# psychopa4/PFNL

Measured on AMD Instinct MI355X. Metric: HR frames/sec at 4xSR, 7-frame 128x128->512x512, higher is better.
Workload: dtype f32

## Files before the change

### pfnl_amd/csrc/nonlocal_f16.hip

```cpp
#include <algorithm>
#include <cstdlib>
#include <type_traits>

#include "common.h"
#include "conv_bf16.h"
#include "conv_split16.h"

namespace pfnl {

typedef _Float16 bf16x8 __attribute__((ext_vector_type(8)));
typedef unsigned u32x4 __attribute__((ext_vector_type(4)));

constexpr int NF_KT = 64;
constexpr int NF_KROW = 208;
constexpr int NF_VROW = 144;
constexpr int NF_CP = 96;
constexpr int NF_THREADS = 512;
constexpr int NF_QB = NF_THREADS / 2;

constexpr float NF_XSCALE = 128.0f;
constexpr float NF_SINV = 1.0f / (128.0f * 128.0f);
constexpr float NF_PSHIFT = 14.0f;
__device__ __forceinline__ unsigned short bf16_bits(float f) {
    const _Float16 b = (_Float16)f;
    return __builtin_bit_cast(unsigned short, b);
}
__device__ __forceinline__ float bf16_float(unsigned short u) { return (float)__builtin_bit_cast(_Float16, u); }

template <bool FROMX>
__global__ __launch_bounds__(256) void nl_pack_f16_kernel(const float* __restrict__ X, uint16_t* __restrict__ Khi, uint16_t* __restrict__ Klo,
                                                          uint16_t* __restrict__ Vthi, uint16_t* __restrict__ Vtlo, int B, int N, int Npad, int C,
                                                          int CPin, const float* __restrict__ xraw, float* __restrict__ Xout, int H, int W) {
    __shared__ uint16_t vth[NF_CP][34], vtl[NF_CP][34];
    const int nblk = Npad / 32;
    const int b = blockIdx.x / nblk, n0 = (blockIdx.x - b * nblk) * 32;
    const int tid = threadIdx.x;
    [[maybe_unused]] const int C3 = C / 4, T = C / 12, W2 = W / 2;
#pragma unroll
    for (int j = 0; j < 32 * NF_CP / 256; ++j) {
        const int i = tid + 256 * j;
        const int kk = i / NF_CP, c = i - kk * NF_CP;
        const int n = n0 + kk;
        float raw = 0.f;
        if constexpr (FROMX) {
            if (n < N && c < C) {
                const int sub = c / C3, k = c - sub * C3;
                const int t = k / 3, cc = k - 3 * t;
                const int y = 2 * (n / W2) + (sub >> 1), xx = 2 * (n % W2) + (sub & 1);
                raw = xraw[((((size_t)b * T + t) * H + y) * W + xx) * 3 + cc];
            }
            if (n < N && c < CPin) Xout[((size_t)b * N + n) * CPin + c] = raw;
        } else {
            raw = (n < N && c < C) ? X[((size_t)b * N + n) * CPin + c] : 0.f;
        }
        const float v = raw * NF_XSCALE;
        const unsigned short hi = bf16_bits(v);
        const unsigned short lo = bf16_bits(v - bf16_float(hi));
        Khi[((size_t)b * Npad + n) * NF_CP + c] = (n >= N && c == C) ? (unsigned short)0xfbff : (c == C + 1 ? (unsigned short)0x3c00 : hi);
        Klo[((size_t)b * Npad + n) * NF_CP + c] = lo;
        const int e = (kk & 3) | (((kk >> 3) & 1) << 2), kh = (kk >> 2) & 1, t = kk >> 4;
        const int pos = 16 * t + 8 * kh + e;
        vth[c][pos] = c == C ? (unsigned short)0x3c00 : hi;
        vtl[c][pos] = c == C ? (unsigned short)0 : lo;
    }
    __syncthreads();
#pragma unroll
    for (int j = 0; j < 16 * NF_CP / 256; ++j) {
        const int i = tid + 256 * j;
        const int c = i >> 4, pp = (i & 15) * 2;
        const size_t vp = ((size_t)b * NF_CP + c) * Npad + n0 + pp;
        *reinterpret_cast<unsigned*>(Vthi + vp) = (unsigned)vth[c][pp] | ((unsigned)vth[c][pp + 1] << 16);
        *reinterpret_cast<unsigned*>(Vtlo + vp) = (unsigned)vtl[c][pp] | ((unsigned)vtl[c][pp + 1] << 16);
    }
}



template <bool SPLIT>
struct NfSW {
    static constexpr int KLO_OFF = NF_KT * NF_KROW;
    static constexpr int VHI_OFF = SPLIT ? 2 * NF_KT * NF_KROW : NF_KT * NF_KROW;
    static constexpr int VLO_OFF = VHI_OFF + NF_CP * NF_VROW;
    static constexpr int TILE_BYTES = SPLIT ? VLO_OFF + NF_CP * NF_VROW : VLO_OFF;
    static constexpr int NSLOT = SPLIT ? 3 : 5;
    static constexpr int PIECES = SPLIT ? 53 : 32;
    static constexpr int SLOT_BYTES = PIECES * 1024;
    static constexpr int PW = (PIECES + 7) / 8;
    static constexpr int LDS_BYTES = NSLOT * SLOT_BYTES;
    static_assert(TILE_BYTES <= SLOT_BYTES && LDS_BYTES <= 160 * 1024, "LDS budget");
    static_assert(SPLIT || PIECES % 8 == 0, "the vmcnt wait of a ring deeper than 3 counts on equal shares");
};

__device__ __forceinline__ void nf_dma16(__amdgpu_buffer_rsrc_t rs, unsigned lds_dst, int voff) {
    unsigned keep;
    asm volatile("s_mov_b32 %0, m0\n\ts_mov_b32 m0, %2\n\ts_nop 0\n\tbuffer_load_dwordx4 %1, %3, 0 offen lds\n\ts_mov_b32 m0, %0"
                 : "=&s"(keep) : "v"(voff), "s"(lds_dst), "s"(rs) : "memory");
}
#define NF_BARRIER() asm volatile("s_waitcnt lgkmcnt(0)\n\ts_barrier" ::: "memory")

template <int C, bool SPLIT>
__global__ __launch_bounds__(NF_THREADS, 2) void nl_attn_f16_sw_kernel(const float* __restrict__ X, const uint16_t* __restrict__ K16,
                                                                 unsigned rel_klo, unsigned rel_vhi, unsigned rel_vlo, unsigned scratch_bytes,
                                                                 float* __restrict__ Xo, const float* __restrict__ Wp,
                                                                 const float* __restrict__ bp, float* __restrict__ Zp,
                                                                 float* __restrict__ ML, int N, int Npad, int q0, int q1) {
    using G = NfSW<SPLIT>;
    constexpr int CT = 3;
    constexpr int CP = (C + 31) / 32 * 32;
    static_assert(C + 1 < NF_CP && C % 2 == 0, "needs two pad channels inside 96");
    extern __shared__ __attribute__((aligned(16))) unsigned char sm[];

    const int tid = threadIdx.x;
    const int lane = tid & 63;
    const int wave = __builtin_amdgcn_readfirstlane(tid >> 6);
    const int xl = lane & 31;
    const int kh = lane >> 5;
    const int b = blockIdx.y;
    const float* Xb = X + (size_t)b * N * CP;
    float* Xob = Xo + (size_t)b * N * CP;
    const int q = q0 + blockIdx.x * NF_QB + (tid >> 6) * 32 + xl;
    const int qc = q < q1 ? q : q1 - 1;

    constexpr float LOG2E = 1.4426950408889634f;
    bf16x8 qh[6];
    [[maybe_unused]] bf16x8 ql[6];
#pragma unroll
    for (int ks = 0; ks < 6; ++ks)
#pragma unroll
        for (int e = 0; e < 8; ++e) {
            const int c = 16 * ks + 8 * kh + e;
            const float v = c < C ? Xb[(size_t)qc * CP + c] * (LOG2E * NF_XSCALE) : (c == C ? 1024.f : 0.f);
            const _Float16 h = (_Float16)v;
            qh[ks][e] = h;
            if constexpr (SPLIT) ql[ks][e] = (_Float16)(v - (float)h);
        }
    constexpr int CS = C;
    constexpr int LCT = CS / 32, LI = CS % 32;
    constexpr int LKH = (LI % 8) >= 4 ? 1 : 0, LR = (LI / 8) * 4 + (LI % 8) % 4;

    f32x16 o[CT];
#pragma unroll
    for (int ct = 0; ct < CT; ++ct)
#pragma unroll
        for (int r = 0; r < 16; ++r) o[ct][r] = 0.f;
    float m = -INFINITY;

    int srel[G::PW];
#pragma unroll
    for (int k = 0; k < G::PW; ++k) {
        const int p = (wave + 8 * k) * 1024 + 16 * lane;
        int sr = 0x7fffffff;
        if (p < NF_KT * NF_KROW || (SPLIT && p < 2 * NF_KT * NF_KROW)) {
            const bool lo = p >= NF_KT * NF_KROW;
            const int r = p - (lo ? NF_KT * NF_KROW : 0);
            const int row = r / NF_KROW, col = r - row * NF_KROW;
            if (col < NF_CP * 2) {
                sr = (int)((lo ? rel_klo : 0u) + (unsigned)(((size_t)b * Npad + row) * (NF_CP * 2)) + col);
            }
        } else if (p < G::TILE_BYTES) {
            const bool lo = SPLIT && p >= G::VLO_OFF;
            const int r = p - (lo ? G::VLO_OFF : G::VHI_OFF);
            const int ch = r / NF_VROW, col = r - ch * NF_VROW;
            if (col < NF_KT * 2) {
                sr = (int)((lo ? rel_vlo : rel_vhi) + (unsigned)(((size_t)b * NF_CP + ch) * Npad * 2) + col);
            }
        }
        srel[k] = sr;
    }
    const unsigned lds0 = (unsigned)(uintptr_t)sm;
    auto tile_piece = [&](int k, int kt, int slot, bool live) __attribute__((always_inline)) {
        const int i = wave + 8 * k;
        if (G::PIECES % 8 == 0 || 8 * k + 7 < G::PIECES || i < G::PIECES) {
            const __amdgpu_buffer_rsrc_t rs = __builtin_amdgcn_make_buffer_rsrc(const_cast<uint16_t*>(K16), 0, live ? scratch_bytes : 0, 0x00020000);
            const int k0 = kt * NF_KT;
            const bool isk = i * 1024 < (SPLIT ? 2 : 1) * NF_KT * NF_KROW;
            const int off = (int)((unsigned)srel[k] + (unsigned)(k0 * (isk ? NF_CP * 2 : 2)));
            nf_dma16(rs, lds0 + slot * G::SLOT_BYTES + i * 1024, off);
        }
    };

    const int ntiles = (N + NF_KT - 1) / NF_KT;
    const int ksp = gridDim.z, sp = blockIdx.z;
    const int kt0 = (int)((long long)ntiles * sp / ksp), kt1 = (int)((long long)ntiles * (sp + 1) / ksp);
#pragma unroll
    for (int j = 0; j < G::NSLOT - 1; ++j)
#pragma unroll
        for (int k = 0; k < G::PW; ++k) tile_piece(k, kt0 + j, j, kt0 + j < kt1);
#pragma unroll
    for (int k = 0; k < G::PW; ++k) tile_piece(k, 0, G::NSLOT - 1, false);
    asm volatile("s_waitcnt vmcnt(0)" ::: "memory");
    __syncthreads();

    bf16x8 pt[2][2];
    [[maybe_unused]] bf16x8 pl[2][2];
#pragma unroll
    for (int i = 0; i < 2; ++i)
#pragma unroll
        for (int j = 0; j < 2; ++j)
#pragma unroll
            for (int e = 0; e < 8; ++e) {
                pt[i][j][e] = (_Float16)0.f;
                if constexpr (SPLIT) pl[i][j][e] = (_Float16)0.f;
            }
#define NP_MFMA(a_, b_, c_) __builtin_amdgcn_mfma_f32_32x32x16_f16(a_, b_, c_, 0, 0, 0)
    f32x16 st[2];
    constexpr int NQ = SPLIT ? 18 : 6, NR = SPLIT ? 24 : 12;
#define NP_PIN(v_) asm volatile("" : "+v"(v_))
    constexpr int AHEAD = 4;
    constexpr int RING = AHEAD + 2;
    bf16x8 rb[RING];
    auto half_body = [&](auto hc, const unsigned char* qbuf, const unsigned char* vbuf, int kt_fill, int s_fill) __attribute__((always_inline)) {
        constexpr int H = decltype(hc)::value;
        f32x16& stc = st[H];
        f32x16& stn = st[H ^ 1];
        const unsigned char* const kah = qbuf + ((1 - H) * 32 + xl) * NF_KROW + kh * 16;
        const unsigned char* const vah = vbuf + G::VHI_OFF + xl * NF_VROW + kh * 16 + (1 - H) * 64;
        auto read = [&](auto qc) __attribute__((always_inline)) {
            constexpr int q = decltype(qc)::value;
            if constexpr (q < NR) {
                constexpr int d = q % RING;
                if constexpr (!SPLIT) {
                    if constexpr (q < 6) rb[d] = *reinterpret_cast<const bf16x8*>(kah + q * 32);
                    else rb[d] = *reinterpret_cast<const bf16x8*>(vah + ((q - 6) % 3) * 32 * NF_VROW + ((q - 6) / 3) * 32);
                } else {
                    if constexpr (q < 12) rb[d] = *reinterpret_cast<const bf16x8*>(kah + (q & 1) * G::KLO_OFF + (q >> 1) * 32);
                    else {
                        constexpr int u = (q - 12) >> 1, lo = (q - 12) & 1;
                        rb[d] = *reinterpret_cast<const bf16x8*>(vah + lo * (G::VLO_OFF - G::VHI_OFF) + (u % 3) * 32 * NF_VROW + (u / 3) * 32);
                    }
                }
            }
        };
        auto mfma = [&](auto ic) __attribute__((always_inline)) {
            constexpr int i = decltype(ic)::value;
            constexpr int q = SPLIT ? 2 * (i / 3) + (i % 3 == 2) : i;
            const bf16x8 a = rb[q % RING];
            if constexpr (i < NQ) {
                constexpr int ks = SPLIT ? i / 3 : i;
                bf16x8 bq = qh[ks];
                if constexpr (SPLIT) {
                    if constexpr (i % 3 == 1) bq = ql[ks];
                }
                if constexpr (i == 0) {
                    f32x16 z;
#pragma unroll
                    for (int r = 0; r < 16; ++r) z[r] = 0.f;
                    stn = NP_MFMA(a, bq, z);
                } else {
                    stn = NP_MFMA(a, bq, stn);
                }
            } else {
                constexpr int j = i - NQ;
                constexpr int u = SPLIT ? j / 3 : j;
                constexpr int jj = u / 3, ct = u % 3;
                bf16x8 bp = pt[1 - H][jj];
                if constexpr (SPLIT) {
                    if constexpr (j % 3 == 1) bp = pl[1 - H][jj];
                }
                o[ct] = NP_MFMA(a, bp, o[ct]);
            }
        };
#pragma unroll
        for (int q0_ = 0; q0_ <= AHEAD; ++q0_) {
            if (q0_ == 0) read(std::integral_constant<int, 0>{});
            if (q0_ == 1) read(std::integral_constant<int, 1>{});
            if (q0_ == 2) read(std::integral_constant<int, 2>{});
            if (q0_ == 3) read(std::integral_constant<int, 3>{});
            if (q0_ == 4) read(std::integral_constant<int, 4>{});
            if (q0_ == 5) read(std::integral_constant<int, 5>{});
            if (q0_ == 6) read(std::integral_constant<int, 6>{});
        }
        __builtin_amdgcn_sched_barrier(0);
        float tmax = 0.f, tsw = 0.f, alpha = 1.f, shift = 0.f;
        [[maybe_unused]] float pv0 = 0.f, pv1 = 0.f;
        auto gap = [&](auto ic) __attribute__((always_inline)) {
            constexpr int i = decltype(ic)::value;
            mfma(ic);
            __builtin_amdgcn_sched_barrier(0);
            {
                constexpr int qn = (SPLIT ? 2 * (i / 3) + (i % 3 == 2) : i) + AHEAD + 1;
                constexpr int qp = i == 0 ? AHEAD + 1 : (SPLIT ? 2 * ((i - 1) / 3) + ((i - 1) % 3 == 2) : i - 1) + AHEAD + 1;
                if constexpr (qn > qp) read(std::integral_constant<int, qn - 1 < NR ? (qn - 1 >= qp ? qn - 1 : NR) : NR>{});
            }
            if constexpr (i == 0) {
                float ta, tb;
                asm("v_max3_f32 %0, %1, %2, %3" : "=v"(ta) : "v"(stc[0]), "v"(stc[1]), "v"(stc[2]));
                asm("v_max3_f32 %0, %1, %2, %3" : "=v"(tb) : "v"(stc[8]), "v"(stc[9]), "v"(stc[10]));
                asm("v_max3_f32 %0, %1, %2, %3" : "=v"(ta) : "v"(ta), "v"(stc[3]), "v"(stc[4]));
                asm("v_max3_f32 %0, %1, %2, %3" : "=v"(tb) : "v"(tb), "v"(stc[11]), "v"(stc[12]));
                asm("v_max3_f32 %0, %1, %2, %3" : "=v"(ta) : "v"(ta), "v"(stc[5]), "v"(stc[6]));
                asm("v_max3_f32 %0, %1, %2, %3" : "=v"(tb) : "v"(tb), "v"(stc[13]), "v"(stc[14]));
                asm("v_max3_f32 %0, %1, %2, %3" : "=v"(ta) : "v"(ta), "v"(stc[7]), "v"(stc[15]));
                asm("v_max_f32 %0, %1, %2" : "=v"(tmax) : "v"(ta), "v"(tb));
                NP_PIN(tmax);
            } else if constexpr (i == 1) {
                tsw = __shfl_xor(tmax, 32);
                NP_PIN(tsw);
            } else if constexpr (i == 3) {
                asm("v_max_f32 %0, %1, %2" : "=v"(tmax) : "v"(tmax), "v"(tsw));
                tmax *= NF_SINV;
                const float mn = fmaxf(m, tmax);
                alpha = __builtin_amdgcn_exp2f(m - mn);
                shift = NF_PSHIFT - mn;
                m = mn;
                NP_PIN(shift);
                NP_PIN(alpha);
            }
            if constexpr (!SPLIT) {
                if constexpr (i >= 4) {
                    constexpr int r = 2 * (i - 4);
                    const float a0 = __builtin_amdgcn_exp2f(__builtin_fmaf(stc[r], NF_SINV, shift));
                    const float a1 = __builtin_amdgcn_exp2f(__builtin_fmaf(stc[r + 1], NF_SINV, shift));
                    pt[H][r >> 3][r & 7] = (_Float16)a0;
                    pt[H][r >> 3][(r & 7) + 1] = (_Float16)a1;
                    NP_PIN(pt[H][r >> 3]);
                }
            } else {
                if constexpr (i >= 4 && i % 2 == 0) {
                    constexpr int r = 2 * ((i - 4) / 4);
                    if constexpr (((i - 4) / 2) % 2 == 0) {
                        pv0 = __builtin_amdgcn_exp2f(__builtin_fmaf(stc[r], NF_SINV, shift));
                        pv1 = __builtin_amdgcn_exp2f(__builtin_fmaf(stc[r + 1], NF_SINV, shift));
                        asm volatile("" : "+v"(pv0), "+v"(pv1));
                    } else {
                        const _Float16 h0 = (_Float16)pv0, h1 = (_Float16)pv1;
                        pt[H][r >> 3][r & 7] = h0;
                        pt[H][r >> 3][(r & 7) + 1] = h1;
                        pl[H][r >> 3][r & 7] = (_Float16)(pv0 - (float)h0);
                        pl[H][r >> 3][(r & 7) + 1] = (_Float16)(pv1 - (float)h1);
                        NP_PIN(pt[H][r >> 3]);
                        NP_PIN(pl[H][r >> 3]);
                    }
                }
            }
            if constexpr (H == 1) {
                constexpr int step = SPLIT ? 5 : 3;
                if constexpr (i % step == 2 && i / step < G::PW) tile_piece(i / step, kt_fill, s_fill, kt_fill < kt1);
            }
            __builtin_amdgcn_sched_barrier(0);
        };
        gap(std::integral_constant<int, 0>{});
        gap(std::integral_constant<int, 1>{});
        gap(std::integral_constant<int, 2>{});
        gap(std::integral_constant<int, 3>{});
        gap(std::integral_constant<int, 4>{});
        gap(std::integral_constant<int, 5>{});
        gap(std::integral_constant<int, 6>{});
        gap(std::integral_constant<int, 7>{});
        gap(std::integral_constant<int, 8>{});
        gap(std::integral_constant<int, 9>{});
        gap(std::integral_constant<int, 10>{});
        gap(std::integral_constant<int, 11>{});
        if constexpr (SPLIT) {
            gap(std::integral_constant<int, 12>{});
            gap(std::integral_constant<int, 13>{});
            gap(std::integral_constant<int, 14>{});
            gap(std::integral_constant<int, 15>{});
            gap(std::integral_constant<int, 16>{});
            gap(std::integral_constant<int, 17>{});
            gap(std::integral_constant<int, 18>{});
            gap(std::integral_constant<int, 19>{});
            gap(std::integral_constant<int, 20>{});
            gap(std::integral_constant<int, 21>{});
            gap(std::integral_constant<int, 22>{});
            gap(std::integral_constant<int, 23>{});
            gap(std::integral_constant<int, 24>{});
            gap(std::integral_constant<int, 25>{});
            gap(std::integral_constant<int, 26>{});
            gap(std::integral_constant<int, 27>{});
            gap(std::integral_constant<int, 28>{});
            gap(std::integral_constant<int, 29>{});
            gap(std::integral_constant<int, 30>{});
            gap(std::integral_constant<int, 31>{});
            gap(std::integral_constant<int, 32>{});
            gap(std::integral_constant<int, 33>{});
            gap(std::integral_constant<int, 34>{});
            gap(std::integral_constant<int, 35>{});
        }
        if (!__all(alpha == 1.0f)) {
#pragma unroll
            for (int ct = 0; ct < CT; ++ct)
#pragma unroll
                for (int r = 0; r < 16; ++r) o[ct][r] *= alpha;
        }
    };

    int s_cur = 0, s_prv = G::NSLOT - 1, s_nxt = 1;
    {
        const unsigned char* const kah = sm + xl * NF_KROW + kh * 16;
#pragma unroll
        for (int r = 0; r < 16; ++r) st[0][r] = 0.f;
#pragma unroll
        for (int ks = 0; ks < 6; ++ks) {
            const bf16x8 ah = *reinterpret_cast<const bf16x8*>(kah + ks * 32);
            st[0] = NP_MFMA(ah, qh[ks], st[0]);
            if constexpr (SPLIT) {
                const bf16x8 al = *reinterpret_cast<const bf16x8*>(kah + G::KLO_OFF + ks * 32);
                st[0] = NP_MFMA(ah, ql[ks], st[0]);
                st[0] = NP_MFMA(al, qh[ks], st[0]);
            }
        }
    }
    for (int kt = kt0; kt < kt1; ++kt) {
        const unsigned char* const cur = sm + s_cur * G::SLOT_BYTES;
        const unsigned char* const prv = sm + s_prv * G::SLOT_BYTES;
        const unsigned char* const nxt = sm + s_nxt * G::SLOT_BYTES;
        half_body(std::integral_constant<int, 0>{}, cur, prv, 0, 0);
        asm volatile("s_waitcnt vmcnt(%0)" ::"n"((G::NSLOT - 3) * G::PW) : "memory");
        NF_BARRIER();
        half_body(std::integral_constant<int, 1>{}, nxt, cur, kt + G::NSLOT - 1, s_prv);
        s_prv = s_cur;
        s_cur = s_nxt;
        s_nxt = s_nxt + 1 == G::NSLOT ? 0 : s_nxt + 1;
    }
    {
        const unsigned char* const vah = sm + s_prv * G::SLOT_BYTES + G::VHI_OFF + xl * NF_VROW + kh * 16 + 64;
#pragma unroll
        for (int jj = 0; jj < 2; ++jj)
#pragma unroll
            for (int ct = 0; ct < CT; ++ct) {
                const bf16x8 vh = *reinterpret_cast<const bf16x8*>(vah + ct * 32 * NF_VROW + jj * 32);
                o[ct] = NP_MFMA(vh, pt[1][jj], o[ct]);
                if constexpr (SPLIT) {
                    const bf16x8 vl = *reinterpret_cast<const bf16x8*>(vah + (G::VLO_OFF - G::VHI_OFF) + ct * 32 * NF_VROW + jj * 32);
                    o[ct] = NP_MFMA(vh, pl[1][jj], o[ct]);
                    o[ct] = NP_MFMA(vl, pt[1][jj], o[ct]);
                }
            }
    }

    float l = o[LCT][LR];
    {
        const float lo = __shfl_xor(l, 32);
        if (kh != LKH) l = lo;
    }
    const float inv = (1.0f / NF_XSCALE) / l;
#pragma unroll
    for (int ct = 0; ct < CT; ++ct)
#pragma unroll
        for (int r = 0; r < 16; ++r) o[ct][r] *= inv;

    constexpr int CTW = CP / 32;
    constexpr int NPAIR = CTW * CTW * 2;
    static_assert(NPAIR * 2048 <= G::SLOT_BYTES * G::NSLOT, "W' in operand form fits the ring");
    asm volatile("s_waitcnt vmcnt(0)" ::: "memory");
    __syncthreads();
    for (int pp = tid; pp < NPAIR * 64; pp += NF_THREADS) {
        const int ln = pp & 63, g = pp >> 6;
        const int t = g & 1, ctp = (g >> 1) % CTW, cotp = (g >> 1) / CTW;
        const float* w = Wp + (size_t)(ctp * 32 + 16 * t + 4 * (ln >> 5)) * CP + cotp * 32 + (ln & 31);
        bf16x8 h, l;
#pragma unroll
        for (int i = 0; i < 8; ++i) {
            const float v = w[((i & 3) + 8 * (i >> 2)) * CP];
            const _Float16 hh = (_Float16)v;
            h[i] = hh;
            l[i] = (_Float16)((v - (float)hh) * 2048.0f);
        }
        *reinterpret_cast<bf16x8*>(sm + g * 2048 + ln * 16) = h;
        *reinterpret_cast<bf16x8*>(sm + g * 2048 + 1024 + ln * 16) = l;
    }
    bf16x8 bh[CTW][2], bl[CTW][2];
#pragma unroll
    for (int ct = 0; ct < CTW; ++ct)
#pragma unroll
        for (int t = 0; t < 2; ++t)
#pragma unroll
            for (int i = 0; i < 8; ++i) {
                const float v = o[ct][8 * t + i];
                const _Float16 hh = (_Float16)v;
                bh[ct][t][i] = hh;
                bl[ct][t][i] = (_Float16)((v - (float)hh) * 2048.0f);
            }
    __syncthreads();
#pragma unroll
    for (int cot = 0; cot < CTW; ++cot) {
        f32x16 z, zc;
#pragma unroll
        for (int r = 0; r < 16; ++r) z[r] = zc[r] = 0.f;
#pragma unroll
        for (int ct = 0; ct < CTW; ++ct)
#pragma unroll
            for (int t = 0; t < 2; ++t) {
                const unsigned char* wa = sm + ((cot * CTW + ct) * 2 + t) * 2048 + lane * 16;
                const bf16x8 ah = *reinterpret_cast<const bf16x8*>(wa), al = *reinterpret_cast<const bf16x8*>(wa + 1024);
                z = NP_MFMA(ah, bh[ct][t], z);
                zc = NP_MFMA(ah, bl[ct][t], zc);
                zc = NP_MFMA(al, bh[ct][t], zc);
            }
#pragma unroll
        for (int r = 0; r < 16; ++r) z[r] = (z[r] + zc[r] * (1.0f / 2048.0f)) * (ksp == 1 ? 1.0f : l);
        if (q < q1) {
            if (ksp == 1) {
#pragma unroll
                for (int r = 0; r < 16; ++r) {
                    const int co = cot * 32 + drow(r, lane);
                    if (co < C) {
                        const size_t idx = (size_t)q * CP + co;
                        Xob[idx] = Xb[idx] + z[r] + bp[co];
                    }
                }
            } else {
                float* zp = Zp + (((size_t)b * ksp + sp) * N + q) * CP;
#pragma unroll
                for (int r = 0; r < 16; ++r) zp[cot * 32 + drow(r, lane)] = z[r];
            }
        }
    }
    if (ksp > 1 && q < q1 && kh == 0) {
        float* ml = ML + (((size_t)b * ksp + sp) * N + q) * 2;
        ml[0] = m;
        ml[1] = l;
    }
}

size_t nl_f16_scratch_halfs(int B, int N) {
    const size_t npad = (size_t)(N + 31) / 32 * 32 + 64;
    return 4 * (size_t)B * NF_CP * npad;
}

static size_t nl_f16_chunk_limit() {
    static const size_t lim = [] {
        const char* e = std::getenv("PFNL_NL_CHUNK_BYTES");
        const long long v = e ? std::atoll(e) : 0;
        return v > 0 ? (size_t)v : (size_t)0x7fff0000ull;
    }();
    return lim;
}

static hipError_t nl_attn_f16_run(const float* X, float* Xo, const float* Wp, const float* bp, float* partial, uint16_t* scratch16,
                                  int B, int N, int C, hipStream_t s, int q0, int q1, bool split, int ks_cap, bool prepacked = false);

bool nl_f16_fits_one_launch(int B, int N) { return 2 * nl_f16_scratch_halfs(1, N) * (size_t)B <= nl_f16_chunk_limit(); }

hipError_t launch_nl_pack_fused(const float* x, float* X, uint16_t* scratch16, int B, int T, int H, int W, hipStream_t s) {
    const int C = 12 * T, N = (H / 2) * (W / 2);
    if (!x || !X || !scratch16 || B < 1 || (C != 84 && C != 60 && C != 36) || (H & 1) || (W & 1) || !nl_f16_fits_one_launch(B, N)) return hipErrorInvalidValue;
    const int CP = nl_padded_ch(C);
    const int npad = (N + 31) / 32 * 32 + 64;
    uint16_t* Khi = scratch16;
    uint16_t* Klo = Khi + (size_t)B * npad * NF_CP;
    uint16_t* Vthi = Klo + (size_t)B * npad * NF_CP;
    uint16_t* Vtlo = Vthi + (size_t)B * NF_CP * npad;
    hipLaunchKernelGGL(nl_pack_f16_kernel<true>, dim3(B * (npad / 32)), dim3(256), 0, s, nullptr, Khi, Klo, Vthi, Vtlo, B, N, npad, C, CP, x, X, H, W);
    return hipGetLastError();
}

hipError_t launch_nl_attn_f16(const float* X, float* Xo, const float* Wp, const float* bp, float* partial, uint16_t* scratch16,
                               int B, int N, int C, hipStream_t s, int q0, int q1, bool split, bool prepacked) {
    if (B < 1 || N < 1) return hipErrorInvalidValue;
    if (prepacked) {
        if (!nl_f16_fits_one_launch(B, N)) return hipErrorInvalidValue;
        return nl_attn_f16_run(X, Xo, Wp, bp, partial, scratch16, B, N, C, s, q0, q1, split, nl_key_splits(B, N), true);
    }
    const size_t per_clip = 2 * nl_f16_scratch_halfs(1, N);
    const int ks_cap = nl_key_splits(B, N);
    int bc = (int)std::min<size_t>((size_t)B, std::max<size_t>(1, nl_f16_chunk_limit() / per_clip));
    const int CP = nl_padded_ch(C);
    for (int b0 = 0; b0 < B; b0 += bc) {
        const int nb = std::min(bc, B - b0);
        hipError_t e = nl_attn_f16_run(X + (size_t)b0 * N * CP, Xo + (size_t)b0 * N * CP, Wp, bp, partial, scratch16, nb, N, C, s, q0, q1, split, ks_cap);
        if (e != hipSuccess) return e;
    }
    return hipSuccess;
}

static hipError_t nl_attn_f16_run(const float* X, float* Xo, const float* Wp, const float* bp, float* partial, uint16_t* scratch16,
                                  int B, int N, int C, hipStream_t s, int q0, int q1, bool split, int ks_cap, bool prepacked) {
    if (C != 84 && C != 60 && C != 36) return hipErrorInvalidValue;
    if (q1 < 0) q1 = N;
    if (q0 < 0 || q0 >= q1 || q1 > N) return hipErrorInvalidValue;
    const int CP = nl_padded_ch(C);
    const int npad = (N + 31) / 32 * 32 + 64;
    uint16_t* Khi = scratch16;
    uint16_t* Klo = Khi + (size_t)B * npad * NF_CP;
    uint16_t* Vthi = Klo + (size_t)B * npad * NF_CP;
    uint16_t* Vtlo = Vthi + (size_t)B * NF_CP * npad;
    if (!prepacked) {
        hipLaunchKernelGGL(nl_pack_f16_kernel<false>, dim3(B * (npad / 32)), dim3(256), 0, s, X, Khi, Klo, Vthi, Vtlo, B, N, npad, C, CP, nullptr, nullptr, 0, 0);
        hipError_t e = hipGetLastError();
        if (e != hipSuccess) return e;
    }
    const int ks_max = std::min(nl_key_splits(B, N), ks_cap);
    int ks = 1;
    {
        const long long qb = (long long)((q1 - q0 + NF_QB - 1) / NF_QB) * B;
        double best = 1e30;
        for (int k = 1; k <= ks_max; ++k) {
            const double t = (double)((qb * k + 255) / 256) / k;
            if (t < best - 1e-9) {
                best = t;
                ks = k;
            }
        }
    }
    if (ks > 1 && !partial) return hipErrorInvalidValue;
    float* Zp = partial;
    float* ML = partial ? partial + (size_t)B * ks * N * CP : nullptr;
    dim3 grid((q1 - q0 + NF_QB - 1) / NF_QB, B, ks);
    dim3 block(NF_THREADS);
    int dev = 0;
    if (hipGetDevice(&dev) != hipSuccess || dev < 0 || dev >= 64) return hipErrorInvalidDevice;
    const size_t scratch_bytes = 2 * nl_f16_scratch_halfs(B, N);
    static std::atomic<int> attr_sw[64];
    if (!attr_sw[dev]) {
        const void* const fns[6] = {
            reinterpret_cast<const void*>(nl_attn_f16_sw_kernel<84, true>), reinterpret_cast<const void*>(nl_attn_f16_sw_kernel<60, true>),
            reinterpret_cast<const void*>(nl_attn_f16_sw_kernel<36, true>), reinterpret_cast<const void*>(nl_attn_f16_sw_kernel<84, false>),
            reinterpret_cast<const void*>(nl_attn_f16_sw_kernel<60, false>), reinterpret_cast<const void*>(nl_attn_f16_sw_kernel<36, false>),
        };
        const int lds[2] = {NfSW<true>::LDS_BYTES, NfSW<false>::LDS_BYTES};
        for (int i = 0; i < 6; ++i) {
            hipError_t e = hipFuncSetAttribute(fns[i], hipFuncAttributeMaxDynamicSharedMemorySize, lds[i / 3]);
            if (e != hipSuccess) return e;
        }
        attr_sw[dev] = 1;
    }
    const unsigned rel_klo = (unsigned)((Klo - Khi) * 2), rel_vhi = (unsigned)((Vthi - Khi) * 2), rel_vlo = (unsigned)((Vtlo - Khi) * 2);
#define NP_LAUNCH(C_, S_) hipLaunchKernelGGL((nl_attn_f16_sw_kernel<C_, S_>), grid, block, (NfSW<S_>::LDS_BYTES), s, X, Khi, rel_klo, rel_vhi, rel_vlo, \
                                             (unsigned)scratch_bytes, Xo, Wp, bp, Zp, ML, N, npad, q0, q1)
    switch (C) {
        case 84: if (split) NP_LAUNCH(84, true); else NP_LAUNCH(84, false); break;
        case 60: if (split) NP_LAUNCH(60, true); else NP_LAUNCH(60, false); break;
        case 36: if (split) NP_LAUNCH(36, true); else NP_LAUNCH(36, false); break;
    }
#undef NP_LAUNCH
    hipError_t e = hipGetLastError();
    if (e != hipSuccess || ks == 1) return e;
    return launch_nl_merge(X, Zp, ML, bp, Xo, B, N, C, ks, s, q0, q1);
}

}
```

Baseline: 936.3.

## Stage fused pack through LDS with vectorized float4 loads and 16-byte stores

Rewrites the FROMX path of the pack kernel so that raw frame pixels are read as coalesced float4 pieces (2 pixels x 6 floats), with a scalar fallback at row or alignment boundaries, and then scattered into a shared-memory tile. The X output, the K hi/lo and the transposed V hi/lo are then written from LDS with 16-byte vector stores instead of per-element 2-byte scattered writes. This is meant to cut the uncoalesced global gather and narrow stores in the space-to-depth pack step. It adds LDS traffic, boundary-case complexity and a new alignment requirement on X and scratch that is checked on the host.

Measured after the change: 935.8 (median of 2 runs). Within noise of the previous version (-0.0%).

```diff
diff --git a/pfnl_amd/csrc/nonlocal_f16.hip b/pfnl_amd/csrc/nonlocal_f16.hip
--- a/pfnl_amd/csrc/nonlocal_f16.hip
+++ b/pfnl_amd/csrc/nonlocal_f16.hip
@@ -27,50 +27,146 @@
 }
 __device__ __forceinline__ float bf16_float(unsigned short u) { return (float)__builtin_bit_cast(_Float16, u); }
 
+constexpr int NP_XS = 100;
+
 template <bool FROMX>
 __global__ __launch_bounds__(256) void nl_pack_f16_kernel(const float* __restrict__ X, uint16_t* __restrict__ Khi, uint16_t* __restrict__ Klo,
                                                           uint16_t* __restrict__ Vthi, uint16_t* __restrict__ Vtlo, int B, int N, int Npad, int C,
                                                           int CPin, const float* __restrict__ xraw, float* __restrict__ Xout, int H, int W) {
-    __shared__ uint16_t vth[NF_CP][34], vtl[NF_CP][34];
     const int nblk = Npad / 32;
     const int b = blockIdx.x / nblk, n0 = (blockIdx.x - b * nblk) * 32;
     const int tid = threadIdx.x;
-    [[maybe_unused]] const int C3 = C / 4, T = C / 12, W2 = W / 2;
-#pragma unroll
-    for (int j = 0; j < 32 * NF_CP / 256; ++j) {
-        const int i = tid + 256 * j;
-        const int kk = i / NF_CP, c = i - kk * NF_CP;
-        const int n = n0 + kk;
-        float raw = 0.f;
-        if constexpr (FROMX) {
-            if (n < N && c < C) {
-                const int sub = c / C3, k = c - sub * C3;
-                const int t = k / 3, cc = k - 3 * t;
-                const int y = 2 * (n / W2) + (sub >> 1), xx = 2 * (n % W2) + (sub & 1);
-                raw = xraw[((((size_t)b * T + t) * H + y) * W + xx) * 3 + cc];
-            }
-            if (n < N && c < CPin) Xout[((size_t)b * N + n) * CPin + c] = raw;
-        } else {
-            raw = (n < N && c < C) ? X[((size_t)b * N + n) * CPin + c] : 0.f;
-        }
-        const float v = raw * NF_XSCALE;
-        const unsigned short hi = bf16_bits(v);
-        const unsigned short lo = bf16_bits(v - bf16_float(hi));
-        Khi[((size_t)b * Npad + n) * NF_CP + c] = (n >= N && c == C) ? (unsigned short)0xfbff : (c == C + 1 ? (unsigned short)0x3c00 : hi);
-        Klo[((size_t)b * Npad + n) * NF_CP + c] = lo;
-        const int e = (kk & 3) | (((kk >> 3) & 1) << 2), kh = (kk >> 2) & 1, t = kk >> 4;
-        const int pos = 16 * t + 8 * kh + e;
-        vth[c][pos] = c == C ? (unsigned short)0x3c00 : hi;
-        vtl[c][pos] = c == C ? (unsigned short)0 : lo;
-    }
-    __syncthreads();
-#pragma unroll
-    for (int j = 0; j < 16 * NF_CP / 256; ++j) {
-        const int i = tid + 256 * j;
-        const int c = i >> 4, pp = (i & 15) * 2;
-        const size_t vp = ((size_t)b * NF_CP + c) * Npad + n0 + pp;
-        *reinterpret_cast<unsigned*>(Vthi + vp) = (unsigned)vth[c][pp] | ((unsigned)vth[c][pp + 1] << 16);
-        *reinterpret_cast<unsigned*>(Vtlo + vp) = (unsigned)vtl[c][pp] | ((unsigned)vtl[c][pp + 1] << 16);
+    if constexpr (FROMX) {
+        __shared__ __attribute__((aligned(16))) float xs[32 * NP_XS];
+        const int T = C / 12, C3 = C / 4, W2 = W / 2;
+        const int nreq = 96 * T;
+        const float4* const safe = reinterpret_cast<const float4*>(xraw + (((0 - reinterpret_cast<uintptr_t>(xraw)) & 15) >> 2));
+        float4 piece[3];
+        bool whole[3];
+#pragma unroll
+        for (int j = 0; j < 3; ++j) {
+            const int i = tid + 256 * j;
+            const int td = i / 48, r = i - td * 48, p = r / 3, q = r - 3 * p;
+            const int n = n0 + 2 * p, row = n / W2, col = n - row * W2;
+            const float* src = xraw + (((size_t)b * T + (td >> 1)) * H + 2 * row + (td & 1)) * W * 3 + (size_t)col * 6 + 4 * q;
+            whole[j] = i < nreq && n + 1 < N && col + 1 < W2 && (reinterpret_cast<uintptr_t>(src) & 15) == 0;
+            piece[j] = *(whole[j] ? reinterpret_cast<const float4*>(src) : safe);
+        }
+#pragma unroll
+        for (int j = 0; j < 3; ++j) {
+            const int i = tid + 256 * j;
+            if (!whole[j] && i < nreq) {
+                const int td = i / 48, r = i - td * 48, p = r / 3, q = r - 3 * p;
+                const int n = n0 + 2 * p, row = n / W2, col = n - row * W2;
+                const float* plane = xraw + ((size_t)b * T + (td >> 1)) * H * W * 3;
+                float e[4];
+#pragma unroll
+                for (int k = 0; k < 4; ++k) {
+                    const int f = 4 * q + k, second = f >= 6 ? 1 : 0;
+                    const int nn = n + second;
+                    const int rr = (second && col + 1 == W2) ? row + 1 : row, cl = second ? (col + 1 == W2 ? 0 : col + 1) : col;
+                    e[k] = nn < N ? plane[((size_t)(2 * rr + (td & 1)) * W + 2 * cl) * 3 + (f - 6 * second)] : 0.f;
+                }
+                piece[j] = make_float4(e[0], e[1], e[2], e[3]);
+            }
+        }
+        const int npc = NF_CP - C;
+        for (int i = tid; i < 32 * npc; i += 256) {
+            const int kk = i / npc;
+            xs[kk * NP_XS + C + (i - kk * npc)] = 0.f;
+        }
+#pragma unroll
+        for (int j = 0; j < 3; ++j) {
+            const int i = tid + 256 * j;
+            if (i < nreq) {
+                const int td = i / 48, r = i - td * 48, p = r / 3, q = r - 3 * p;
+                const float e[4] = {piece[j].x, piece[j].y, piece[j].z, piece[j].w};
+#pragma unroll
+                for (int k = 0; k < 4; ++k) {
+                    const int f = 4 * q + k, second = f >= 6 ? 1 : 0, w = f - 6 * second, dx = w >= 3 ? 1 : 0;
+                    xs[(2 * p + second) * NP_XS + ((td & 1) * 2 + dx) * C3 + 3 * (td >> 1) + (w - 3 * dx)] = e[k];
+                }
+            }
+        }
+        __syncthreads();
+        const int cp4 = CPin / 4;
+        for (int i = tid; i < 32 * cp4; i += 256) {
+            const int kk = i / cp4, q = i - kk * cp4;
+            if (n0 + kk < N)
+                *reinterpret_cast<float4*>(Xout + ((size_t)b * N + n0 + kk) * CPin + 4 * q) = *reinterpret_cast<const float4*>(xs + kk * NP_XS + 4 * q);
+        }
+        for (int u = tid; u < 32 * (NF_CP / 8); u += 256) {
+            const int kk = u / (NF_CP / 8), g = u - kk * (NF_CP / 8);
+            const int n = n0 + kk;
+            const float4 r0 = *reinterpret_cast<const float4*>(xs + kk * NP_XS + 8 * g), r1 = *reinterpret_cast<const float4*>(xs + kk * NP_XS + 8 * g + 4);
+            const float raw[8] = {r0.x, r0.y, r0.z, r0.w, r1.x, r1.y, r1.z, r1.w};
+            unsigned short hi[8], lo[8];
+#pragma unroll
+            for (int e = 0; e < 8; ++e) {
+                const int c = 8 * g + e;
+                const float v = raw[e] * NF_XSCALE;
+                const unsigned short h = bf16_bits(v);
+                lo[e] = bf16_bits(v - bf16_float(h));
+                hi[e] = (n >= N && c == C) ? (unsigned short)0xfbff : (c == C + 1 ? (unsigned short)0x3c00 : h);
+            }
+            u32x4 ph, pl;
+#pragma unroll
+            for (int e = 0; e < 4; ++e) {
+                ph[e] = (unsigned)hi[2 * e] | ((unsigned)hi[2 * e + 1] << 16);
+                pl[e] = (unsigned)lo[2 * e] | ((unsigned)lo[2 * e + 1] << 16);
+            }
+            const size_t kp = ((size_t)b * Npad + n) * NF_CP + 8 * g;
+            *reinterpret_cast<u32x4*>(Khi + kp) = ph;
+            *reinterpret_cast<u32x4*>(Klo + kp) = pl;
+        }
+        for (int u = tid; u < NF_CP * 4; u += 256) {
+            const int c = u >> 2, j = u & 3;
+            const int kb = 16 * (j >> 1) + 4 * (j & 1);
+            unsigned short hi[8], lo[8];
+#pragma unroll
+            for (int e = 0; e < 8; ++e) {
+                const float v = xs[(kb + (e & 3) + ((e >> 2) << 3)) * NP_XS + c] * NF_XSCALE;
+                const unsigned short h = bf16_bits(v);
+                hi[e] = c == C ? (unsigned short)0x3c00 : h;
+                lo[e] = c == C ? (unsigned short)0 : bf16_bits(v - bf16_float(h));
+            }
+            u32x4 ph, pl;
+#pragma unroll
+            for (int e = 0; e < 4; ++e) {
+                ph[e] = (unsigned)hi[2 * e] | ((unsigned)hi[2 * e + 1] << 16);
+                pl[e] = (unsigned)lo[2 * e] | ((unsigned)lo[2 * e + 1] << 16);
+            }
+            const size_t vp = ((size_t)b * NF_CP + c) * Npad + n0 + 8 * j;
+            *reinterpret_cast<u32x4*>(Vthi + vp) = ph;
+            *reinterpret_cast<u32x4*>(Vtlo + vp) = pl;
+        }
+    } else {
+        __shared__ uint16_t vth[NF_CP][34], vtl[NF_CP][34];
+#pragma unroll
+        for (int j = 0; j < 32 * NF_CP / 256; ++j) {
+            const int i = tid + 256 * j;
+            const int kk = i / NF_CP, c = i - kk * NF_CP;
+            const int n = n0 + kk;
+            const float raw = (n < N && c < C) ? X[((size_t)b * N + n) * CPin + c] : 0.f;
+            const float v = raw * NF_XSCALE;
+            const unsigned short hi = bf16_bits(v);
+            const unsigned short lo = bf16_bits(v - bf16_float(hi));
+            Khi[((size_t)b * Npad + n) * NF_CP + c] = (n >= N && c == C) ? (unsigned short)0xfbff : (c == C + 1 ? (unsigned short)0x3c00 : hi);
+            Klo[((size_t)b * Npad + n) * NF_CP + c] = lo;
+            const int e = (kk & 3) | (((kk >> 3) & 1) << 2), kh = (kk >> 2) & 1, t = kk >> 4;
+            const int pos = 16 * t + 8 * kh + e;
+            vth[c][pos] = c == C ? (unsigned short)0x3c00 : hi;
+            vtl[c][pos] = c == C ? (unsigned short)0 : lo;
+        }
+        __syncthreads();
+#pragma unroll
+        for (int j = 0; j < 16 * NF_CP / 256; ++j) {
+            const int i = tid + 256 * j;
+            const int c = i >> 4, pp = (i & 15) * 2;
+            const size_t vp = ((size_t)b * NF_CP + c) * Npad + n0 + pp;
+            *reinterpret_cast<unsigned*>(Vthi + vp) = (unsigned)vth[c][pp] | ((unsigned)vth[c][pp + 1] << 16);
+            *reinterpret_cast<unsigned*>(Vtlo + vp) = (unsigned)vtl[c][pp] | ((unsigned)vtl[c][pp + 1] << 16);
+        }
     }
 }
 
@@ -542,6 +638,7 @@
     uint16_t* Klo = Khi + (size_t)B * npad * NF_CP;
     uint16_t* Vthi = Klo + (size_t)B * npad * NF_CP;
     uint16_t* Vtlo = Vthi + (size_t)B * NF_CP * npad;
+    if ((reinterpret_cast<uintptr_t>(X) | reinterpret_cast<uintptr_t>(scratch16)) & 15) return hipErrorInvalidValue;
     hipLaunchKernelGGL(nl_pack_f16_kernel<true>, dim3(B * (npad / 32)), dim3(256), 0, s, nullptr, Khi, Klo, Vthi, Vtlo, B, N, npad, C, CP, x, X, H, W);
     return hipGetLastError();
 }
```
